# causalflow-ai/petit-kernel

Measured on AMD Instinct MI355X. Metric: bf16xnvfp4_gemm_achieved_hbm_bandwidth_m1_n8192_k8192, higher is better.
Workload: dtype bf16; 1 GPU; M=1 N=8192 K=8192 bf16 x nvfp4 (e4m3 scales, g=16), one mul_nvfp4_a16 call per step; weights_rotated_over_copies=37, parallelism=replicas x1 (no data-path collective), launch=hip graph replay (1 replays per region), statistic=one region, warmup_steps_run=4000

## Files before the change

### petit-kernel_amd/csrc/gemm_native32.hpp

```cpp
#pragma once

#include "gemm_native.hpp"
#include "gemm_wide.hpp"

#ifndef PETIT_ABLATE_N32
#define PETIT_ABLATE_N32 0
#endif

namespace petit_amd {

template <int ACT> __host__ __device__ inline size_t native32_ws_bytes(unsigned m, unsigned k) {
    return (size_t)m * (k / 8 * ACT) + (size_t)m * (k / 32);
}

struct QuantGather {
    const int *idx;
    unsigned a_rows, xb;
};
__device__ __forceinline__ unsigned q_row() { return blockIdx.y; }
__device__ __forceinline__ unsigned q_row(const QuantGather &g) { return blockIdx.x / g.xb; }
__device__ __forceinline__ unsigned q_bx() { return blockIdx.x; }
__device__ __forceinline__ unsigned q_bx(const QuantGather &g) { return blockIdx.x % g.xb; }
__device__ __forceinline__ unsigned q_src(unsigned row) { return row; }
__device__ __forceinline__ unsigned q_src(unsigned row, const QuantGather &g) { return g.idx ? (unsigned)g.idx[row] : row; }
// ... 295 lines not shown
    static constexpr int kSmemU4 = (kSmemU4a > kRedU4 ? kSmemU4a : kRedU4) + 16 * PW;
    static_assert(kSmemU4 * 16 <= 160 * 1024, "LDS budget");
    static constexpr int kMinWavesPerSimd = (kWantTwoPerSimd && (KG == 2 || kSmemU4 * 16 <= 80 * 1024)) ? 2 : 1;
};

constexpr int n32_stage_refills(bool last_span, int t_first, int kt, int d, int ks, int np, int wloads = 2) {
    if (t_first < 0)
        return wloads * np * kt;
    int n = 0;
    for (int t = t_first; t < t_first + kt; ++t)
        n += (!last_span || t + d < ks) ? wloads * np : 0;
    return n;
}

template <class Cfg, class... Moe>
__global__ __launch_bounds__(Cfg::kThreads, Cfg::kMinWavesPerSimd) void gemm_native32_kernel(const GemmArgs p, const unsigned char *ws,
                                                                                             const Moe... moe) {
    static_assert(sizeof...(Moe) <= 1, "at most one MoE locator");
    constexpr bool kIdx = sizeof...(Moe) == 1;
    using AT = typename Cfg::AT;
    constexpr int KS = Cfg::KS, MB = Cfg::MB, NP = Cfg::NP, WAVES = Cfg::WAVES, D = Cfg::D, ACT = Cfg::ACT;
    constexpr int KT = Cfg::KT, PF = Cfg::PF, NBUF = Cfg::NBUF, WM = Cfg::WM, kWaves = Cfg::kWaves;
    constexpr unsigned kRecBytes = ScaleRec<kFmtMx, KS>::kBytes;
    constexpr int kRecDw = ScaleRec<kFmtMx, KS>::kDwords;
    constexpr unsigned kOob = 0x80000000u;
    constexpr int kFragU4 = ACT == 4 ? 1 : 2;
    constexpr int kBlgp = ACT == 8 ? 0 : ACT == 6 ? 2 : 4;
    constexpr int WF = Cfg::WF, kWL = Cfg::kWLoads;
    constexpr int kCbsz = WF == 6 ? 2 : 4;

    __shared__ u32x4 smem[Cfg::kSmemU4];

    constexpr int KG = Cfg::KG;
    const unsigned tid = threadIdx.x;
    const unsigned lane = tid & 63u;
    const unsigned wave_all = __builtin_amdgcn_readfirstlane(tid >> 6);
    const unsigned kg = KG == 1 ? 0u : wave_all / kWaves;
    const unsigned wave = KG == 1 ? wave_all : wave_all % kWaves;
    const unsigned wn = WM == 1 ? wave : wave % WAVES, wm = WM == 1 ? 0u : wave / WAVES;
    const unsigned m_l = lane & 31u, h = lane >> 5;
    u32x4 *const smem_g = smem + kg * (NBUF * Cfg::kStageU4);

    const unsigned ktiles = p.k / kTileK;
    const unsigned nspans = ktiles / KS;
    const unsigned ntiles = p.n / kTileN;
    unsigned bn, bm, m0, m_lim = p.m;
    const void *w_e = p.w, *s_e = p.s, *bias_e = p.bias;
    const float *gs_e = p.gs;
    RowIndex ix{};
    if constexpr (kIdx) {
        if (!(moe.locate(p, bn, m0, m_lim, w_e, s_e, gs_e, bias_e, ix) && ...))
            return;
    } else {
        tile_of_block(p.flags, bn, bm);
    }
    const unsigned nt0 = (bn * WAVES + wn) * (2 * NP);
    if constexpr (!kIdx)
        m0 = bm * Cfg::BM;
    const unsigned part_begin = (blockIdx.z * KG + kg) * p.spans_per_wave;
    const bool empty_part = KG == 2 && part_begin >= nspans;
    const unsigned sp_begin = min(part_begin, nspans - 1);
    const unsigned sp_end = min(sp_begin + p.spans_per_wave, nspans);
    const unsigned kt_begin = sp_begin * KS;

    f32x16 acc[MB][NP];
#pragma unroll
    for (int mb = 0; mb < MB; ++mb)
#pragma unroll
        for (int np = 0; np < NP; ++np)
#pragma unroll
            for (int v = 0; v < 16; ++v)
                acc[mb][np][v] = 0.f;

    const unsigned valid_nt = (nt0 < ntiles && !empty_part) ? min((unsigned)(2 * NP), ntiles - nt0) : 0u;
    const unsigned w_row_bytes = ktiles * kTileBytes;
    const unsigned s_row_bytes = p.k / 2;
    const unsigned rows = min(m_lim - m0, (unsigned)Cfg::BM);
    const unsigned pt0 = valid_nt ? physical_tile(nt0, ntiles, p.act) : 0u;
    const unsigned span_tiles = !valid_nt ? 0u : p.act ? (valid_nt >> 1) + (ntiles >> 1) : valid_nt;
    const __amdgpu_buffer_rsrc_t w_rsrc = WF == 6 ? make_rsrc(w_e, (unsigned)nv6_elem_bytes(p.n, p.k))
                                                  : make_rsrc((const char *)w_e + (size_t)pt0 * w_row_bytes, span_tiles * w_row_bytes);
    const __amdgpu_buffer_rsrc_t s_rsrc = WF == 6 ? make_rsrc(s_e, (unsigned)nv6_scale_bytes(p.n, p.k))
                                                  : make_rsrc((const char *)s_e + (size_t)pt0 * s_row_bytes, span_tiles * s_row_bytes);
    unsigned w_voff[2 * NP], s_voff[2 * NP];
    if constexpr (WF == 6) {
#pragma unroll
        for (int np = 0; np < NP; ++np) {
            const unsigned nt = 2 * np + (m_l >> 4);
            const unsigned pt = physical_tile(nt0 + nt, ntiles, p.act);
            const unsigned lane_img = h * 32 + (pt & 1u) * 16 + (m_l & 15u);
            w_voff[np] = nt < valid_nt ? (pt >> 1) * (ktiles * kNv6TileBytes) + lane_img * 16 : kOob;
            s_voff[np] = nt < valid_nt ? (pt >> 1) * (ktiles * 128u) + lane_img * (2 * KS) : kOob;
        }
    } else {
#pragma unroll
        for (int nt = 0; nt < 2 * NP; ++nt) {
            const unsigned rel = physical_tile(nt0 + nt, ntiles, p.act) - pt0;
            w_voff[nt] = ((unsigned)nt < valid_nt) ? lane * 16 + rel * w_row_bytes : kOob;
            s_voff[nt] = ((unsigned)nt < valid_nt) ? lane * kRecBytes + rel * s_row_bytes : kOob;
        }
    }
    auto w_load = [&](int i, unsigned kt) -> u32x4 {
        if constexpr (WF == 6)
            return buf_load16(w_rsrc, w_voff[i / 3], kt * kNv6TileBytes + (i % 3) * 1024u, kAuxDefault);
        else
            return buf_load16(w_rsrc, w_voff[i], kt * kTileBytes, kAuxDefault);
    };
    constexpr unsigned kRowB = 16 * Cfg::kRowU4;
    const size_t qa_bytes = (size_t)p.m * (p.k / 8 * ACT), qs_bytes = (size_t)p.m * (p.k / 32);
    const size_t lo_bytes = (size_t)p.m * (p.k / 8 * Cfg::kRowU4);
    const __amdgpu_buffer_rsrc_t qa_rsrc = make_rsrc(ws + (size_t)m0 * kRowB, (unsigned)(lo_bytes - (size_t)m0 * kRowB));
    const __amdgpu_buffer_rsrc_t qh_rsrc = make_rsrc(ws + lo_bytes + (size_t)m0 * 32, ACT == 6 ? (unsigned)(qa_bytes - lo_bytes - (size_t)m0 * 32) : 0u);
    const __amdgpu_buffer_rsrc_t qs_rsrc = make_rsrc(ws + qa_bytes + (size_t)m0 * 4, (unsigned)(qs_bytes - (size_t)m0 * 4));
    const unsigned qa_tile = p.m * kRowB, qs_tile = p.m * 4;

    constexpr unsigned U = Cfg::kRowU4, RPL = Cfg::kRowsPerLoad;
    constexpr int kDmaWaves = Cfg::kDmaWaves;
    const bool dma_wave = kDmaWaves == kWaves || wave < (unsigned)kDmaWaves;
    const unsigned dma_row0 = wave * RPL + lane / U;
    auto swz = [](unsigned row) -> unsigned { return ACT == 8 ? (row >> 1) & 7u : (row >> 2) & 3u; };
    const unsigned hi_row0 = wave * 32 + (lane >> 1);
    const unsigned hi_voff = (ACT == 6 && dma_wave) ? hi_row0 * 32 + (((lane & 1u) ^ ((hi_row0 >> 3) & 1u)) * 16) : kOob;
    const unsigned dma_voff = dma_wave ? dma_row0 * kRowB + (((lane % U) ^ swz(dma_row0)) * 16) : kOob;
    const unsigned qs_voff = (wave * 64 < (unsigned)Cfg::BM) ? (wave * 64 + lane) * 4 : kOob;
    auto dma_stage = [&](unsigned kt, unsigned buf) {
#if defined(__HIP_DEVICE_COMPILE__) && !(PETIT_ABLATE_N32 & 1)
#pragma unroll
        for (int t = 0; t < KT; ++t) {
            u32x4 *const data = smem_g + buf * Cfg::kStageU4 + t * Cfg::kDataU4;
            u32x4 *const dump = smem_g + buf * Cfg::kStageU4 + KT * (Cfg::kDataU4 + Cfg::kScaleU4);
#pragma unroll
            for (int i = 0; i < Cfg::kDataLoads; ++i)
                __builtin_amdgcn_raw_ptr_buffer_load_lds(qa_rsrc, (__attribute__((address_space(3))) void *)(dma_wave ? data + (i * kDmaWaves + wave) * 64 : dump), 16,
                                                         dma_voff, i * (RPL * kDmaWaves) * kRowB + (kt + t) * qa_tile, 0, 0);
            if constexpr (ACT == 6) {
#pragma unroll
                for (int i = 0; i < Cfg::kHiLoads; ++i)
                    __builtin_amdgcn_raw_ptr_buffer_load_lds(qh_rsrc, (__attribute__((address_space(3))) void *)(dma_wave ? data + Cfg::kLoU4 + (i * kDmaWaves + wave) * 64 : dump), 16,
                                                             hi_voff, i * (32 * kDmaWaves) * 32 + (kt + t) * (p.m * 32), 0, 0);
            }
            u32x4 *const sc = smem_g + buf * Cfg::kStageU4 + KT * Cfg::kDataU4 + t * Cfg::kScaleU4;
            __builtin_amdgcn_raw_ptr_buffer_load_lds(qs_rsrc, (__attribute__((address_space(3))) void *)(sc + wave * 16), 4, qs_voff, (kt + t) * qs_tile, 0, 0);
        }
#else
        (void)kt, (void)buf;
#endif
    };
    struct Frags {
        u32x4 d[MB][kFragU4];
        int s[MB];
    };
    struct Frag1 {
        u32x4 d[kFragU4];
        int s;
    };
    const unsigned my_swz = swz(m_l);
    const unsigned hi_swz = (m_l >> 3) & 1u;
    auto read_frag1 = [&](const u32x4 *a_cur, const unsigned char *sc_bytes, int q, int mb, Frag1 &f) {
        const unsigned row = (wm * MB + mb) * 32 + m_l;
        if constexpr (ACT == 6) {
            f.d[0] = a_cur[row * U + ((2 * q + h) ^ my_swz)];
            if (q == 0)
                f.d[1] = a_cur[Cfg::kLoU4 + row * 2 + (h ^ hi_swz)];
        } else {
#pragma unroll
            for (int e = 0; e < kFragU4; ++e) {
                const unsigned unit = ACT == 8 ? 4 * q + 2 * h + e : 2 * q + h;
                f.d[e] = a_cur[row * U + (unit ^ my_swz)];
            }
        }
        f.s = (int)sc_bytes[row * 4 + 2 * q + h];
    };
    auto read_frags = [&](const u32x4 *a_cur, const unsigned char *sc_bytes, int q, Frags &f) {
#pragma unroll
        for (int mb = 0; mb < MB; ++mb) {
            const unsigned row = (wm * MB + mb) * 32 + m_l;
            if constexpr (ACT == 6) {
                f.d[mb][0] = a_cur[row * U + ((2 * q + h) ^ my_swz)];
                if (q == 0)
                    f.d[mb][1] = a_cur[Cfg::kLoU4 + row * 2 + (h ^ hi_swz)];
            } else {
#pragma unroll
                for (int e = 0; e < kFragU4; ++e) {
                    const unsigned unit = ACT == 8 ? 4 * q + 2 * h + e : 2 * q + h;
                    f.d[mb][e] = a_cur[row * U + (unit ^ my_swz)];
                }
            }
            f.s[mb] = (int)sc_bytes[row * 4 + 2 * q + h];
        }
// ... 30 lines not shown
#pragma unroll
            for (int i = 0; i < PF; ++i)
                load_stage(kt_begin + i * KT, i);
            asm volatile("s_waitcnt vmcnt(0)" ::: "memory");
            __builtin_amdgcn_s_barrier();
            const unsigned nstages = (sp_end - sp_begin) * (KS / KT);
            unsigned buf = PF % NBUF;
            for (unsigned st = 0; st < nstages; ++st) {
                load_stage(kt_begin + (st + PF) * KT, buf);
                buf = buf == (unsigned)(NBUF - 1) ? 0u : buf + 1;
                if (st + 1 < nstages) {
                    asm volatile("s_waitcnt vmcnt(%0)" ::"n"((PF - 1) * kLdStage) : "memory");
                    __builtin_amdgcn_s_barrier();
                }
            }
            asm volatile("s_waitcnt vmcnt(0)" ::: "memory");
#endif
            return;
        }
        if constexpr (Cfg::PW) {
            if (wave_all == (unsigned)(kWaves * KG + 1)) {
#if defined(__HIP_DEVICE_COMPILE__)
                constexpr int kPwTiles = 2 * NP * WAVES, kPwLoads = (kPwTiles * 8 + 63) / 64, kAhead = PETIT_N32_PW;
                const unsigned nt0_wg = bn * WAVES * (2 * NP);
                const unsigned valid_wg = nt0_wg < ntiles ? min((unsigned)kPwTiles, ntiles - nt0_wg) : 0u;
                const unsigned pt0_wg = valid_wg ? physical_tile(nt0_wg, ntiles, p.act) : 0u;
                const unsigned span_wg = !valid_wg ? 0u : p.act ? (valid_wg >> 1) + (ntiles >> 1) : valid_wg;
                const __amdgpu_buffer_rsrc_t pw_rsrc = make_rsrc((const char *)w_e + (size_t)pt0_wg * w_row_bytes, span_wg * w_row_bytes);
                u32x4 *const pw_dump = smem + (Cfg::kSmemU4 - 16);
                unsigned pvoff[kPwLoads];
#pragma unroll
                for (int j = 0; j < kPwLoads; ++j) {
                    const unsigned idx = j * 64 + lane, t = idx / 8, line = idx % 8;
                    const bool mine = PETIT_N32_PWSHARE == 1 || (idx % PETIT_N32_PWSHARE) == ((m0 / Cfg::BM) % PETIT_N32_PWSHARE);
                    pvoff[j] = (t < valid_wg && mine) ? (physical_tile(nt0_wg + t, ntiles, p.act) - pt0_wg) * w_row_bytes + line * 128 : kOob;
                }
                auto prefetch = [&](unsigned kt) {
                    if (kt < kt_end) {
#pragma unroll
                        for (int j = 0; j < kPwLoads; ++j)
                            __builtin_amdgcn_raw_ptr_buffer_load_lds(pw_rsrc, (__attribute__((address_space(3))) void *)pw_dump, 4, pvoff[j], kt * kTileBytes, 0, 0);
                    }
                };
                for (unsigned kt = kt_begin + D; kt < kt_begin + kAhead; ++kt)
                    prefetch(kt);
                __builtin_amdgcn_s_barrier();
                const unsigned nstages = (sp_end - sp_begin) * (KS / KT);
                for (unsigned st = 0; st < nstages; ++st) {
#pragma unroll
                    for (int t = 0; t < KT; ++t)
                        prefetch(kt_begin + st * KT + t + kAhead);
                    if (st + 1 < nstages)
                        __builtin_amdgcn_s_barrier();
                }
                asm volatile("s_waitcnt vmcnt(0)" ::: "memory");
#endif
                return;
            }
        }
    } else {
        dma_stage(kt_begin, 0);
#pragma unroll
        for (int i = 1; i < PF; ++i)
            if (kt_begin + i * KT < kt_end)
                dma_stage(kt_begin + i * KT, i);
    }
    ScaleRec<kFmtMx, KS> rec[NP][2], rec_next[NP][2];
    auto load_recs = [&](ScaleRec<kFmtMx, KS> (*dst)[2], unsigned sp) {
        if constexpr (WF == 6) {
#pragma unroll
            for (int np = 0; np < NP; ++np) {
                const ScaleRec<kFmtNv, KS> x = load_scale_rec<kFmtNv, KS>(s_rsrc, s_voff[np], sp * 64 * (2 * KS));
                if constexpr (KS == 2) {
                    dst[np][0].d[0] = x.d[0] & 0xffffu, dst[np][1].d[0] = x.d[0] >> 16;
                } else {
#pragma unroll
                    for (int d = 0; d < kRecDw; ++d)
                        dst[np][0].d[d] = x.d[d], dst[np][1].d[d] = x.d[kRecDw + d];
                }
            }
            return;
        }
#pragma unroll
        for (int np = 0; np < NP; ++np) {
            const ScaleRec<kFmtMx, KS> x = load_scale_rec<kFmtMx, KS>(s_rsrc, s_voff[2 * np], sp * 64 * kRecBytes);
            const ScaleRec<kFmtMx, KS> y = load_scale_rec<kFmtMx, KS>(s_rsrc, s_voff[2 * np + 1], sp * 64 * kRecBytes);
#pragma unroll
            for (int d = 0; d < kRecDw; ++d)
                merge_tiles(x.d[d], y.d[d], dst[np][0].d[d], dst[np][1].d[d]);
        }
    };
    load_recs(rec, sp_begin);
    u32x4 wring[D][kWL * NP];
#pragma unroll
    for (int i = 0; i < D; ++i)
#pragma unroll
        for (int nt = 0; nt < kWL * NP; ++nt)
            wring[i][nt] = w_load(nt, kt_begin + i);
    __syncthreads();

    unsigned cur_buf = 0;
    auto span_body = [&](const unsigned sp, auto last_c) {
        constexpr bool kLast = decltype(last_c)::value;
        const unsigned kt0 = sp * KS;
        if constexpr (!kLast)
            load_recs(rec_next, sp + 1);
        static_for<0, KS / KT>([&](auto s_c) {
            constexpr int S = decltype(s_c)::value, T0 = S * KT;
            constexpr bool kNextStage = !kLast || (T0 + KT < KS);
            const unsigned kt = kt0 + T0;
            const u32x4 *const stage = smem_g + cur_buf * Cfg::kStageU4;
            const unsigned char *const stage_sc = reinterpret_cast<const unsigned char *>(stage + KT * Cfg::kDataU4);
            if constexpr (PF == 1) {
                if constexpr (kNextStage)
                    dma_stage(kt + KT, cur_buf ^ 1u);
            } else {
                if constexpr (!Cfg::LW)
                    dma_stage(kt + PF * KT, cur_buf == 0 ? (unsigned)(NBUF - 1) : cur_buf - 1);
            }
            Frags fr[Cfg::kLean ? 1 : 2];
            Frag1 f1[2];
            unsigned tail_keep[MB][2];
            if constexpr (Cfg::kLean)
                read_frag1(stage, stage_sc, 0, 0, f1[0]);
            else
                read_frags(stage, stage_sc, 0, fr[0]);
            __builtin_amdgcn_sched_barrier(0);
            int refills = 0;
            static_for<0, KT>([&](auto t_c) {
                constexpr int TI = decltype(t_c)::value, T = T0 + TI, SLOT = T % D;
                constexpr bool kRefill = !kLast || (T + D < KS);
                const u32x4 *const a_cur = stage + TI * Cfg::kDataU4;
                const unsigned char *const sc_cur = stage_sc + TI * Cfg::kScaleU4 * 16;
                i32x8 wop[NP][2];
#pragma unroll
                for (int np = 0; np < NP; ++np) {
                    if constexpr (WF == 6) {
                        const u32x4 l1 = wring[SLOT][3 * np], l2 = wring[SLOT][3 * np + 1], tl = wring[SLOT][3 * np + 2];
                        wop[np][0] = i32x8{(int)l1[0], (int)l1[1], (int)l1[2], (int)l1[3], (int)tl[0], (int)tl[1], 0, 0};
                        wop[np][1] = i32x8{(int)l2[0], (int)l2[1], (int)l2[2], (int)l2[3], (int)tl[2], (int)tl[3], 0, 0};
                    } else {
                        unsigned pw[2][4];
#pragma unroll
                        for (int j = 0; j < 4; ++j)
                            merge_tiles(wring[SLOT][2 * np][j], wring[SLOT][2 * np + 1][j], pw[0][j], pw[1][j]);
#pragma unroll
                        for (int q = 0; q < 2; ++q)
                            wop[np][q] = i32x8{(int)pw[q][0], (int)pw[q][1], (int)pw[q][2], (int)pw[q][3], 0, 0, 0, 0};
                    }
                }
                auto refill_slot = [&]() {
                    if constexpr (kRefill && !(PETIT_ABLATE_N32 & 2)) {
#pragma unroll
                        for (int nt = 0; nt < kWL * NP; ++nt)
                            wring[SLOT][nt] = w_load(nt, kt0 + T + D);
                    }
                };
                if constexpr (WF != 6)
                    refill_slot();
                static_for<0, 2>([&](auto q_c) {
                    constexpr int q = decltype(q_c)::value, gi = 2 * TI + q;
                    if constexpr (Cfg::kLean) {
                        static_for<0, MB>([&](auto mb_c) {
                            constexpr int mb = decltype(mb_c)::value, li = gi * MB + mb;
                            if constexpr (li + 1 < 2 * KT * MB) {
                                constexpr int ngi = (li + 1) / MB, nmb = (li + 1) % MB, nti = ngi / 2, nq = ngi % 2;
                                read_frag1(stage + nti * Cfg::kDataU4, stage_sc + nti * Cfg::kScaleU4 * 16, nq, nmb, f1[(li + 1) & 1]);
                            }
                            const u32x4 lo = f1[li & 1].d[0], hi = f1[li & 1].d[kFragU4 - 1];
                            i32x8 aop;
                            if constexpr (ACT == 6) {
                                if constexpr (q == 0) {
                                    tail_keep[mb][0] = hi[2], tail_keep[mb][1] = hi[3];
                                    aop = i32x8{(int)lo[0], (int)lo[1], (int)lo[2], (int)lo[3], (int)hi[0], (int)hi[1], 0, 0};
                                } else {
                                    aop = i32x8{(int)lo[0], (int)lo[1], (int)lo[2], (int)lo[3], (int)tail_keep[mb][0], (int)tail_keep[mb][1], 0, 0};
                                }
                            } else {
                                aop = i32x8{(int)lo[0], (int)lo[1], (int)lo[2], (int)lo[3], (int)hi[0], (int)hi[1], (int)hi[2], (int)hi[3]};
                            }
#pragma unroll
                            for (int np = 0; np < NP; ++np)
                                acc[mb][np] = __builtin_amdgcn_mfma_scale_f32_32x32x64_f8f6f4(wop[np][q], aop, acc[mb][np], kCbsz , kBlgp ,
                                                                                              T % 4, (int)rec[np][q].d[T / 4], 0, f1[li & 1].s);
                        });
                    }
                    if constexpr (!Cfg::kLean && gi + 1 < 2 * KT && !(PETIT_ABLATE_N32 & 4)) {
                        constexpr int nti = (gi + 1) / 2, nq = (gi + 1) % 2;
                        read_frags(stage + nti * Cfg::kDataU4, stage_sc + nti * Cfg::kScaleU4 * 16, nq, fr[(gi + 1) & 1]);
                        if constexpr (ACT == 6 && nq == 1) {
#pragma unroll
                            for (int mb = 0; mb < MB; ++mb)
                                fr[1].d[mb][1] = fr[0].d[mb][1];
                        }
                    }
#pragma unroll
                    for (int mb = 0; mb < (Cfg::kLean ? 0 : MB); ++mb) {
                        i32x8 aop;
                        constexpr int fi = (PETIT_ABLATE_N32 & 4) ? 0 : (Cfg::kLean ? 0 : (gi & 1));
                        if constexpr (ACT == 8) {
                            const u32x4 lo = fr[fi].d[mb][0], hi = fr[fi].d[mb][kFragU4 - 1];
                            aop = i32x8{(int)lo[0], (int)lo[1], (int)lo[2], (int)lo[3], (int)hi[0], (int)hi[1], (int)hi[2], (int)hi[3]};
                        } else if constexpr (ACT == 6) {
                            const u32x4 lo = fr[fi].d[mb][0], tail = fr[fi].d[mb][1];
                            aop = i32x8{(int)lo[0], (int)lo[1], (int)lo[2], (int)lo[3], (int)tail[2 * q], (int)tail[2 * q + 1], 0, 0};
                        } else {
                            const u32x4 lo = fr[fi].d[mb][0];
                            aop = i32x8{(int)lo[0], (int)lo[1], (int)lo[2], (int)lo[3], 0, 0, 0, 0};
                        }
#pragma unroll
                        for (int np = 0; np < NP; ++np) {
                            if constexpr (PETIT_ABLATE_N32 & 8) {
#if defined(__HIP_DEVICE_COMPILE__)
                                asm volatile("" ::"v"(wop[np][q]), "v"(aop), "v"(fr[fi].s[mb]), "v"(rec[np][q].d[T / 4]));
#endif
                            } else {
                                acc[mb][np] = __builtin_amdgcn_mfma_scale_f32_32x32x64_f8f6f4(
                                    wop[np][q], aop, acc[mb][np], kCbsz , kBlgp , T % 4,
                                    (int)rec[np][q].d[T / 4], 0, fr[fi].s[mb]);
                            }
                        }
                    }
                    __builtin_amdgcn_sched_barrier(0);
                });
                if constexpr (WF == 6) {
                    refill_slot();
                    __builtin_amdgcn_sched_barrier(0);
                }
                (void)a_cur, (void)sc_cur, (void)refills;
            });
            if constexpr (PF == 1) {
                if constexpr (kNextStage)
                    __syncthreads();
                cur_buf ^= 1u;
            } else {
                if constexpr (kNextStage) {
                    constexpr int kPrevRefills = [] {
                        int n = 0;
                        for (int j = 1; j < PF; ++j)
                            n += n32_stage_refills(kLast, T0 - j * KT, KT, D, KS, NP, Cfg::kWLoads);
                        n += n32_stage_refills(kLast, T0, KT, D, KS, NP, Cfg::kWLoads);
                        return (PETIT_ABLATE_N32 & 2) ? 0 : n;
                    }();
#if defined(__HIP_DEVICE_COMPILE__)
                    if constexpr (!Cfg::LW)
                        asm volatile("s_waitcnt vmcnt(%0)" ::"n"((PF - 1) * Cfg::kStageLoads + kPrevRefills) : "memory");
                    __builtin_amdgcn_s_barrier();
#endif
                }
                __builtin_amdgcn_sched_barrier(0);
                cur_buf = cur_buf == (unsigned)(NBUF - 1) ? 0u : cur_buf + 1;
            }
            __builtin_amdgcn_sched_barrier(0);
        });
        if constexpr (!kLast) {
#pragma unroll
            for (int np = 0; np < NP; ++np)
                rec[np][0] = rec_next[np][0], rec[np][1] = rec_next[np][1];
        }
    };
    for (unsigned sp = sp_begin; sp + 1 < sp_end; ++sp)
        span_body(sp, std::false_type{});
    span_body(sp_end - 1, std::true_type{});

#pragma unroll
    for (int mb = 0; mb < MB; ++mb)
#pragma unroll
        for (int np = 0; np < NP; ++np) {
#if defined(__HIP_DEVICE_COMPILE__)
            asm volatile("" : "+v"(acc[mb][np]));
#endif
        }

    if constexpr (KG == 2) {
        for (unsigned i = sp_end - sp_begin; i < p.spans_per_wave; ++i)
            for (int b = 0; b < KS / KT; ++b)
                __builtin_amdgcn_s_barrier();
        __syncthreads();
        float *const red = reinterpret_cast<float *>(smem);
        if (kg == 1) {
#pragma unroll
            for (int mb = 0; mb < MB; ++mb)
#pragma unroll
                for (int np = 0; np < NP; ++np)
#pragma unroll
                    for (int v = 0; v < 16; ++v)
                        red[(((wn * MB + mb) * NP + np) * 16 + v) * 64 + lane] = acc[mb][np][v];
        }
        __syncthreads();
        if (kg == 0) {
#pragma unroll
            for (int mb = 0; mb < MB; ++mb)
#pragma unroll
                for (int np = 0; np < NP; ++np)
#pragma unroll
                    for (int v = 0; v < 16; ++v)
                        acc[mb][np][v] += red[(((wn * MB + mb) * NP + np) * 16 + v) * 64 + lane];
        }
    }

    if constexpr (PETIT_ABLATE_N32 & 16)
        return;
    const unsigned m_base = m0 + wm * (32 * MB) + m_l;
    if (gridDim.z > 1) {
        if (KG == 2 && kg != 0)
            return;
#pragma unroll
        for (int mb = 0; mb < MB; ++mb)
#pragma unroll
            for (int np = 0; np < NP; ++np)
#pragma unroll
// ... 73 lines not shown
```

### petit-kernel_amd/csrc/gemm_wide.hpp

```cpp
#pragma once

#include "gemm_tiled.hpp"

namespace petit_amd {

typedef __attribute__((ext_vector_type(16))) float f32x16;

#ifndef PETIT_ABLATE
#define PETIT_ABLATE 0
#endif

__device__ __forceinline__ f32x16 mfma32(bf16x8 a, bf16x8 b, f32x16 c) {
    return __builtin_amdgcn_mfma_f32_32x32x16_bf16(a, b, c, 0, 0, 0);
}
__device__ __forceinline__ f32x16 mfma32(f16x8 a, f16x8 b, f32x16 c) {
    return __builtin_amdgcn_mfma_f32_32x32x16_f16(a, b, c, 0, 0, 0);
}

__device__ __forceinline__ void pin_here(unsigned &x) {
#if defined(__HIP_DEVICE_COMPILE__)
    asm volatile("" : "+v"(x));
#endif
}
__device__ __forceinline__ void pin_here(u32x4 &x) {
// ... 4 lines not shown

__device__ __forceinline__ void merge_tiles(unsigned x, unsigned y, unsigned &p1, unsigned &p2) {
    const auto a = __builtin_amdgcn_permlane16_swap(x, y, false, false);
    const unsigned a0 = a[0], a1 = a[1];
    const auto b = __builtin_amdgcn_permlane32_swap(a0, a1, false, false);
    p1 = b[0], p2 = b[1];
}

template <class AT_, int FMT_, int KS_, int MB_, int NP_, int WAVES_, int D_, int PF_ = 1, int KG_ = 1, int GA_ = 0> struct WideCfg {
    using AT = AT_;
    static constexpr int GA = GA_;
    static_assert(GA_ == 0 || (KG_ == 1 && PF_ == 1 && !AT_::kAdaptive), "group-ahead form: one K group, double-buffered A tile, plain 16-bit activations");
    static constexpr int FMT = FMT_, KS = KS_, MB = MB_, NP = NP_, WAVES = WAVES_, D = D_, PF = PF_, NBUF = PF_ + 1, KG = KG_;
    static constexpr int kThreads = 64 * WAVES * KG;
    static constexpr int BM = 32 * MB, BN = 32 * NP * WAVES;
    static constexpr int kBufU4 = BM * 16;
    static constexpr int kDmaLoads = BM * 16 / 64 / WAVES;
    static constexpr int kMinWavesPerSimd = (KG == 2 || (NP == 1 && MB <= 4 && PF == 1)) ? 2 : 1;
    static constexpr int kRedU4 = KG == 2 ? BM * BN / 4 : 0;
    static constexpr int kSmemU4 = KG * NBUF * kBufU4 > kRedU4 ? KG * NBUF * kBufU4 : kRedU4;
    static_assert(KG == 1 || KG == 2, "one or two K groups");
    static_assert(PF == 1 || PF == 2, "prefetch distance 1 or 2");
    static_assert(!AT::kBfp, "plain bf16 / fp16 activations (or Fp16Mx: fast body + exact fallback, device_common.hpp)");
    static_assert(!AT::kAdaptive || FMT == kFmtMx, "Fp16Mx: fp16 activations x MXFP4 weights");
    static_assert(KS % D == 0, "ring depth must divide the span");
    static_assert((BM * 16) % (64 * WAVES) == 0 && (4 * WAVES) % 16 == 0, "A tile must split into whole 16-row groups per wave-load");
    static_assert(kSmemU4 * 16 <= 160 * 1024, "LDS budget");
};

template <class Cfg>
__global__ __launch_bounds__(Cfg::kThreads, Cfg::kMinWavesPerSimd) void gemm_wide_kernel(const GemmArgs p) {
    using AT = typename Cfg::AT;
    using Frag = typename AT::frag;
    constexpr int FMT = Cfg::FMT, KS = Cfg::KS, MB = Cfg::MB, NP = Cfg::NP, WAVES = Cfg::WAVES, D = Cfg::D;
    constexpr int PF = Cfg::PF, NBUF = Cfg::NBUF;
    constexpr unsigned kRecBytes = ScaleRec<FMT, KS>::kBytes;
    constexpr int kRecDw = ScaleRec<FMT, KS>::kDwords;
    constexpr unsigned kOob = 0x80000000u;

    constexpr int KG = Cfg::KG;
    __shared__ u32x4 smem_all[Cfg::kSmemU4];

    const unsigned tid = threadIdx.x;
    const unsigned lane = tid & 63u;
    const unsigned wave_all = __builtin_amdgcn_readfirstlane(tid >> 6);
    const unsigned kg = KG == 1 ? 0u : wave_all / WAVES;
    const unsigned wave = KG == 1 ? wave_all : wave_all % WAVES;
    u32x4 *const smem = smem_all + kg * (NBUF * Cfg::kBufU4);
    const unsigned m_l = lane & 31u, h = lane >> 5;

    const unsigned ktiles = p.k / kTileK;
    const unsigned nspans = ktiles / KS;
    const unsigned ntiles = p.n / kTileN;
    unsigned bn, bm;
    tile_of_block(p.flags, bn, bm);
    stagger_priority(p.flags);
    const unsigned nt0 = (bn * WAVES + wave) * (2 * NP);
    const unsigned m0 = bm * Cfg::BM;
    const unsigned part_begin = (blockIdx.z * KG + kg) * p.spans_per_wave;
    const bool empty_part = KG == 2 && part_begin >= nspans;
    const unsigned sp_begin = min(part_begin, nspans - 1);
    const unsigned sp_end = min(sp_begin + p.spans_per_wave, nspans);
    const unsigned kt_begin = sp_begin * KS;

    f32x16 acc[MB][NP];
#pragma unroll
    for (int mb = 0; mb < MB; ++mb)
#pragma unroll
        for (int np = 0; np < NP; ++np)
#pragma unroll
            for (int v = 0; v < 16; ++v)
                acc[mb][np][v] = 0.f;

    const unsigned valid_nt = (nt0 < ntiles && !empty_part) ? min((unsigned)(2 * NP), ntiles - nt0) : 0u;
    const unsigned w_row_bytes = ktiles * kTileBytes;
    const unsigned s_row_bytes = (FMT == kFmtNv) ? p.k : p.k / 2;
    const unsigned rows = min(p.m - m0, (unsigned)Cfg::BM);
    const unsigned pt0 = valid_nt ? physical_tile(nt0, ntiles, p.act) : 0u;
    const unsigned span_tiles = !valid_nt ? 0u : p.act ? (valid_nt >> 1) + (ntiles >> 1) : valid_nt;
    const __amdgpu_buffer_rsrc_t w_rsrc = make_rsrc((const char *)p.w + (size_t)pt0 * w_row_bytes, span_tiles * w_row_bytes);
    const __amdgpu_buffer_rsrc_t s_rsrc = make_rsrc((const char *)p.s + (size_t)pt0 * s_row_bytes, span_tiles * s_row_bytes);
    const __amdgpu_buffer_rsrc_t a_rsrc = make_rsrc((const char *)p.a + (size_t)m0 * p.k * 2, rows * p.k * 2);

    unsigned w_voff[2 * NP], s_voff[2 * NP];
#pragma unroll
    for (int nt = 0; nt < 2 * NP; ++nt) {
        const unsigned rel = physical_tile(nt0 + nt, ntiles, p.act) - pt0;
        w_voff[nt] = ((unsigned)nt < valid_nt) ? lane * 16 + rel * w_row_bytes : kOob;
        s_voff[nt] = ((unsigned)nt < valid_nt) ? lane * kRecBytes + rel * s_row_bytes : kOob;
    }
    const unsigned dma_row0 = wave * 4 + (lane >> 4);
    const unsigned dma_voff = dma_row0 * p.k * 2 + (((lane & 15u) ^ (dma_row0 & 15u)) * 16);
    auto dma_a_tile = [&](u32x4 *dst, unsigned kt) {
#pragma unroll
        for (int i = 0; i < Cfg::kDmaLoads; ++i) {
#if defined(__HIP_DEVICE_COMPILE__)
            __builtin_amdgcn_raw_ptr_buffer_load_lds(a_rsrc, (__attribute__((address_space(3))) void *)(dst + (i * WAVES + wave) * 64),
                                                     16, dma_voff, i * (4 * WAVES) * p.k * 2 + kt * 256, 0, 0);
#else
            (void)dst, (void)kt;
#endif
        }
    };
    const unsigned frag_row = m_l * 16, frag_swz = m_l & 15u;
    auto read_frags = [&](const u32x4 *a_cur, int g, u32x4 *dst) {
        const int q = g >> 2, j = g & 3;
#pragma unroll
        for (int mb = 0; mb < MB; ++mb)
            dst[mb] = a_cur[mb * 32 * 16 + frag_row + ((unsigned)(8 * q + 4 * h + j) ^ frag_swz)];
    };

    bool mx_fb = false;
    if constexpr (AT::kAdaptive) {
        const unsigned range = (sp_end - sp_begin) * 64u * kRecBytes;
        unsigned bad = 0;
#pragma unroll
        for (int nt = 0; nt < 2 * NP; ++nt) {
            if ((unsigned)nt >= valid_nt)
                continue;
            const unsigned row0 = s_voff[nt] - lane * kRecBytes + sp_begin * 64u * kRecBytes;
#pragma unroll 4
            for (unsigned base = 0; base < range; base += 1024u) {
                const unsigned off = base + lane * 16u;
                const u32x4 v = __builtin_bit_cast(u32x4, __builtin_amdgcn_raw_buffer_load_b128(s_rsrc, off < range ? row0 + off : kOob, 0, kAuxDefault));
                unsigned t = 0;
#pragma unroll
                for (int d = 0; d < 4; ++d) {
                    const unsigned x = v[d];
                    t |= (0x8C8C8C8Cu - x) | (x - 0x72727272u);
                }
                bad |= off < range ? t : 0u;
            }
        }
        mx_fb = __builtin_amdgcn_ballot_w64((bad & 0xE0E0E0E0u) != 0) != 0;
    }

    const unsigned kt_end = sp_end * KS;
    dma_a_tile(smem, kt_begin);
    if constexpr (PF == 2) {
        if (kt_begin + 1 < kt_end)
            dma_a_tile(smem + Cfg::kBufU4, kt_begin + 1);
    }
    if (AT::kAdaptive && mx_fb) {
        if constexpr (AT::kAdaptive) {
            __syncthreads();
            unsigned rel = 0;
#pragma unroll 1
            for (unsigned kt = kt_begin; kt < kt_end; ++kt) {
                const u32x4 *const a_cur = smem + rel * Cfg::kBufU4;
                if constexpr (PF == 1) {
                    if (kt + 1 < kt_end)
                        dma_a_tile(smem + (rel ^ 1u) * Cfg::kBufU4, kt + 1);
                } else {
                    dma_a_tile(smem + (rel == 0 ? 2u : rel - 1) * Cfg::kBufU4, kt + 2);
                }
#pragma unroll
                for (int np = 0; np < NP; ++np) {
                    const u32x4 x = buf_load16(w_rsrc, w_voff[2 * np], kt * kTileBytes, kAuxDefault);
                    const u32x4 y = buf_load16(w_rsrc, w_voff[2 * np + 1], kt * kTileBytes, kAuxDefault);
                    float sc[2];
#pragma unroll
                    for (int q = 0; q < 2; ++q) {
                        const unsigned tile = (lane >> 4) & 1u, src_lane = 16u * (2u * q + (lane >> 5)) + (lane & 15u);
                        const unsigned voff = s_voff[2 * np] == kOob ? kOob : s_voff[2 * np] - lane * kRecBytes + src_lane * kRecBytes + kt % KS;
                        const unsigned voff_y = s_voff[2 * np + 1] == kOob ? kOob : s_voff[2 * np + 1] - lane * kRecBytes + src_lane * kRecBytes + kt % KS;
                        const unsigned sb = __builtin_amdgcn_raw_buffer_load_b8(s_rsrc, tile ? voff_y : voff, (kt / KS) * 64 * kRecBytes, kAuxDefault);
                        sc[q] = __builtin_bit_cast(float, (sb & 0xffu) << 23);
                    }
#pragma unroll
                    for (int j = 0; j < 4; ++j) {
                        unsigned p[2];
                        merge_tiles(x[j], y[j], p[0], p[1]);
#pragma unroll
                        for (int q = 0; q < 2; ++q) {
                            const bf16x8 wb = unpack_mx(Bf16{}, p[q], sc[q]);
#pragma unroll
                            for (int mb = 0; mb < MB; ++mb) {
                                u32x4 hi, lo;
                                split_f16(a_cur[mb * 32 * 16 + frag_row + ((unsigned)(8 * q + 4 * h + j) ^ frag_swz)], hi, lo);
                                acc[mb][np] = mfma32(wb, __builtin_bit_cast(bf16x8, hi), acc[mb][np]);
                                acc[mb][np] = mfma32(wb, __builtin_bit_cast(bf16x8, lo), acc[mb][np]);
                            }
                        }
                    }
                }
                if (kt + 1 < kt_end)
                    __syncthreads();
                rel = rel + 1 == (unsigned)NBUF ? 0u : rel + 1;
            }
        }
    } else {
    ScaleRec<FMT, KS> rec[NP][2], rec_next[NP][2];
    auto load_recs = [&](ScaleRec<FMT, KS> (*dst)[2], unsigned sp) {
#pragma unroll
        for (int np = 0; np < NP; ++np) {
            const ScaleRec<FMT, KS> x = load_scale_rec<FMT, KS>(s_rsrc, s_voff[2 * np], sp * 64 * kRecBytes);
            const ScaleRec<FMT, KS> y = load_scale_rec<FMT, KS>(s_rsrc, s_voff[2 * np + 1], sp * 64 * kRecBytes);
#pragma unroll
            for (int d = 0; d < kRecDw; ++d)
                merge_tiles(x.d[d], y.d[d], dst[np][0].d[d], dst[np][1].d[d]);
        }
    };
    load_recs(rec, sp_begin);
    u32x4 wring[D][2 * NP];
#pragma unroll
    for (int i = 0; i < D; ++i)
#pragma unroll
        for (int nt = 0; nt < 2 * NP; ++nt)
            wring[i][nt] = buf_load16(w_rsrc, w_voff[nt], (kt_begin + i) * kTileBytes, kAuxDefault);

    if constexpr (Cfg::GA) {
    Frag wfg[2][NP];
    unsigned pw2[NP][4];
    auto unpack_ga = [&](auto c_c, auto slot_c, auto t_c, const ScaleRec<FMT, KS> (*rc)[2]) {
        constexpr int C = decltype(c_c)::value, SLOT = decltype(slot_c)::value, TS = decltype(t_c)::value, j = C % 4, q = C / 4;
#pragma unroll
        for (int np = 0; np < NP; ++np) {
            unsigned w;
            if constexpr (q == 0) {
                unsigned x = wring[SLOT][2 * np][j], y = wring[SLOT][2 * np + 1][j];
                pin_here(x), pin_here(y);
                merge_tiles(x, y, w, pw2[np][j]);
            } else {
                w = pw2[np][j];
                pin_here(w);
            }
            float s_lo, s_hi;
            tile_scales<FMT, KS, TS>(rc[np][q], s_lo, s_hi);
            Frag f;
            if constexpr (PETIT_ABLATE & 4)
                f = __builtin_bit_cast(Frag, u32x4{w, w ^ __builtin_bit_cast(unsigned, s_lo), w, __builtin_bit_cast(unsigned, s_hi)});
            else if constexpr (FMT == kFmtNv)
                f = unpack_nv(AT{}, w, j < 2 ? s_lo : s_hi);
            else
                f = unpack_mx(AT{}, w, s_lo);
            u32x4 fb = __builtin_bit_cast(u32x4, f);
            pin_here(fb);
            wfg[C & 1][np] = __builtin_bit_cast(Frag, fb);
        }
    };
    unpack_ga(std::integral_constant<int, 0>{}, std::integral_constant<int, 0>{}, std::integral_constant<int, 0>{}, rec);
    __syncthreads();
    auto span_body = [&](const unsigned sp, auto last_c) {
        constexpr bool kLast = decltype(last_c)::value;
        const unsigned kt0 = sp * KS;
        if constexpr (!kLast)
            load_recs(rec_next, sp + 1);
        static_for<0, KS>([&](auto t_c) {
            constexpr int T = decltype(t_c)::value;
            constexpr int SLOT = T % D, NSLOT = (T + 1) % D;
            constexpr bool kNext = !kLast || (T + 1 < KS);
            constexpr bool kRefill = !kLast || (T + D < KS);
            constexpr int TN = (T + 1) % KS;
            const unsigned kt = kt0 + T;
            const u32x4 *const a_cur = smem + (T & 1) * Cfg::kBufU4;
            u32x4 *const a_pf = smem + ((T + 1) & 1) * Cfg::kBufU4;
            if constexpr (kNext && !(PETIT_ABLATE & 1))
                dma_a_tile(a_pf, kt + 1);
            u32x4 fr[2][MB];
            read_frags(a_cur, 0, fr[0]);
            if constexpr (PETIT_ABLATE & 8)
                read_frags(a_cur, 1, fr[1]);
            __builtin_amdgcn_sched_barrier(0);
            static_for<0, 8>([&](auto g_c) {
                constexpr int g = decltype(g_c)::value;
                if constexpr (g + 1 < 8 && !(PETIT_ABLATE & 8))
                    read_frags(a_cur, g + 1, fr[(g + 1) & 1]);
#pragma unroll
                for (int mb = 0; mb < MB; ++mb)
#pragma unroll
                    for (int np = 0; np < NP; ++np)
                        acc[mb][np] = mfma32(wfg[g & 1][np], __builtin_bit_cast(Frag, fr[g & 1][mb]), acc[mb][np]);
                if constexpr (g + 1 < 8) {
                    unpack_ga(std::integral_constant<int, g + 1>{}, std::integral_constant<int, SLOT>{}, t_c, rec);
                } else if constexpr (kNext) {
                    if constexpr (TN == 0)
                        unpack_ga(std::integral_constant<int, 0>{}, std::integral_constant<int, NSLOT>{}, std::integral_constant<int, 0>{}, rec_next);
                    else
                        unpack_ga(std::integral_constant<int, 0>{}, std::integral_constant<int, NSLOT>{}, std::integral_constant<int, TN>{}, rec);
                }
                if constexpr (g == 2 && kRefill && !(PETIT_ABLATE & 2)) {
#pragma unroll
                    for (int nt = 0; nt < 2 * NP; ++nt)
                        wring[SLOT][nt] = buf_load16(w_rsrc, w_voff[nt], (kt + D) * kTileBytes, kAuxDefault);
                }
                __builtin_amdgcn_sched_barrier(0);
            });
            if constexpr (kNext && !(PETIT_ABLATE & 32))
                __syncthreads();
        });
        if constexpr (!kLast) {
#pragma unroll
            for (int np = 0; np < NP; ++np)
                rec[np][0] = rec_next[np][0], rec[np][1] = rec_next[np][1];
        }
    };
    for (unsigned sp = sp_begin; sp + 1 < sp_end; ++sp)
        span_body(sp, std::false_type{});
    span_body(sp_end - 1, std::true_type{});
    } else {
    Frag wf[2][NP][2][4];
    unsigned pw2[NP][4];
    auto unpack_chunk = [&](auto c_c, auto slot_c, auto buf_c, auto t_c, const ScaleRec<FMT, KS> (*rc)[2]) {
        constexpr int C = decltype(c_c)::value, SLOT = decltype(slot_c)::value, BUF = decltype(buf_c)::value;
        constexpr int TS = decltype(t_c)::value, j = C % 4, q = C / 4;
#pragma unroll
        for (int np = 0; np < NP; ++np) {
            unsigned w;
            if constexpr (q == 0) {
                unsigned x = wring[SLOT][2 * np][j], y = wring[SLOT][2 * np + 1][j];
                pin_here(x), pin_here(y);
                merge_tiles(x, y, w, pw2[np][j]);
            } else {
                w = pw2[np][j];
                pin_here(w);
            }
            float s_lo, s_hi;
            tile_scales<FMT, KS, TS>(rc[np][q], s_lo, s_hi);
            Frag f;
            if constexpr (PETIT_ABLATE & 4)
                f = __builtin_bit_cast(Frag, u32x4{w, w ^ __builtin_bit_cast(unsigned, s_lo), w, __builtin_bit_cast(unsigned, s_hi)});
            else if constexpr (FMT == kFmtNv)
                f = unpack_nv(AT{}, w, j < 2 ? s_lo : s_hi);
            else
                f = unpack_mx(AT{}, w, s_lo);
            u32x4 fb = __builtin_bit_cast(u32x4, f);
            pin_here(fb);
            wf[BUF][np][q][j] = __builtin_bit_cast(Frag, fb);
        }
    };
    static_for<0, 8>([&](auto c_c) {
        unpack_chunk(c_c, std::integral_constant<int, 0>{}, std::integral_constant<int, 0>{}, std::integral_constant<int, 0>{}, rec);
    });
    if (kt_begin + D < kt_end) {
#pragma unroll
        for (int nt = 0; nt < 2 * NP; ++nt)
            wring[0][nt] = buf_load16(w_rsrc, w_voff[nt], (kt_begin + D) * kTileBytes, kAuxDefault);
    }
    __syncthreads();

    unsigned rel3 = 0;
    auto span_body = [&](const unsigned sp, auto last_c) {
        constexpr bool kLast = decltype(last_c)::value;
        const unsigned kt0 = sp * KS;
        if constexpr (!kLast)
            load_recs(rec_next, sp + 1);
        static_for<0, KS>([&](auto t_c) {
            constexpr int T = decltype(t_c)::value;
            constexpr int CUR = T % 2, NXT = (T + 1) % 2;
            constexpr int NSLOT = (T + 1) % D;
            constexpr bool kNext = !kLast || (T + 1 < KS);
            constexpr bool kRefill = !kLast || (T + 1 + D < KS);
            constexpr int TN = (T + 1) % KS;
            const unsigned kt = kt0 + T;
            unsigned cur_buf, pf_buf;
            if constexpr (NBUF == 2) {
                cur_buf = T & 1, pf_buf = (T + 1) & 1;
            } else {
                cur_buf = rel3, pf_buf = rel3 == 0 ? 2u : rel3 - 1;
            }
            const u32x4 *const a_cur = smem + cur_buf * Cfg::kBufU4;
            u32x4 *const a_pf = smem + pf_buf * Cfg::kBufU4;
            if constexpr (PETIT_ABLATE & 1) {
            } else if constexpr (PF == 1) {
                if constexpr (kNext)
                    dma_a_tile(a_pf, kt + 1);
            } else {
                dma_a_tile(a_pf, kt + 2);
            }
            u32x4 fr[2][MB];
            read_frags(a_cur, 0, fr[0]);
            __builtin_amdgcn_sched_barrier(0);
            static_for<0, 8>([&](auto g_c) {
                constexpr int g = decltype(g_c)::value;
                if constexpr (g + 1 < 8 && !(PETIT_ABLATE & 8))
                    read_frags(a_cur, g + 1, fr[(g + 1) & 1]);
                constexpr int q = g >> 2, j = g & 3;
#pragma unroll
                for (int mb = 0; mb < MB; ++mb)
#pragma unroll
                    for (int np = 0; np < NP; ++np)
                        if constexpr (PETIT_ABLATE & 16) {
                            const u32x4 wb = __builtin_bit_cast(u32x4, wf[CUR][np][q][j]), ab = fr[(PETIT_ABLATE & 8) ? 0 : (g & 1)][mb];
                            acc[mb][np][g] += __builtin_bit_cast(float, wb[0] ^ ab[1]);
                        } else {
                            acc[mb][np] = mfma32(wf[CUR][np][q][j], __builtin_bit_cast(Frag, fr[(PETIT_ABLATE & 8) ? 0 : (g & 1)][mb]), acc[mb][np]);
                        }
                if constexpr (kNext) {
                    if constexpr (TN == 0)
                        unpack_chunk(g_c, std::integral_constant<int, NSLOT>{}, std::integral_constant<int, NXT>{},
                                     std::integral_constant<int, 0>{}, rec_next);
                    else
                        unpack_chunk(g_c, std::integral_constant<int, NSLOT>{}, std::integral_constant<int, NXT>{},
                                     std::integral_constant<int, TN>{}, rec);
                }
                __builtin_amdgcn_sched_barrier(0);
            });
            if constexpr (PF == 1) {
                if constexpr (kRefill && !(PETIT_ABLATE & 2)) {
#pragma unroll
                    for (int nt = 0; nt < 2 * NP; ++nt)
                        wring[NSLOT][nt] = buf_load16(w_rsrc, w_voff[nt], (kt + 1 + D) * kTileBytes, kAuxDefault);
                }
                if constexpr (kNext && !(PETIT_ABLATE & 1))
                    __syncthreads();
            } else {
                if constexpr (kNext) {
#if defined(__HIP_DEVICE_COMPILE__)
                    asm volatile("s_waitcnt vmcnt(%0)" ::"n"(Cfg::kDmaLoads) : "memory");
                    __builtin_amdgcn_s_barrier();
#endif
                }
                __builtin_amdgcn_sched_barrier(0);
                if constexpr (kRefill) {
#pragma unroll
                    for (int nt = 0; nt < 2 * NP; ++nt)
                        wring[NSLOT][nt] = buf_load16(w_rsrc, w_voff[nt], (kt + 1 + D) * kTileBytes, kAuxDefault);
                }
                rel3 = rel3 == 2 ? 0u : rel3 + 1;
            }
        });
        if constexpr (!kLast) {
#pragma unroll
            for (int np = 0; np < NP; ++np)
                rec[np][0] = rec_next[np][0], rec[np][1] = rec_next[np][1];
        }
    };
    for (unsigned sp = sp_begin; sp + 1 < sp_end; ++sp)
        span_body(sp, std::false_type{});
    span_body(sp_end - 1, std::true_type{});
    }
    }
    if constexpr (AT::kAdaptive) {
        static_for<0, 2>([&](auto pass) {
#pragma unroll
            for (int mb = 0; mb < MB; ++mb)
#pragma unroll
                for (int np = 0; np < NP; ++np)
                    mfma_join_pin(acc[mb][np]);
            if constexpr (decltype(pass)::value == 0)
                mfma_join_settle();
        });
    }

    if constexpr (KG == 2) {
        for (unsigned i = sp_end - sp_begin; i < p.spans_per_wave; ++i)
            for (int b = 0; b < KS; ++b)
                __builtin_amdgcn_s_barrier();
        __syncthreads();
        float *const red = reinterpret_cast<float *>(smem_all);
        if (kg == 1) {
#pragma unroll
            for (int mb = 0; mb < MB; ++mb)
#pragma unroll
                for (int np = 0; np < NP; ++np)
#pragma unroll
                    for (int v = 0; v < 16; ++v)
                        red[(((wave * MB + mb) * NP + np) * 16 + v) * 64 + lane] = acc[mb][np][v];
        }
        __syncthreads();
        if (kg == 1)
            return;
#pragma unroll
        for (int mb = 0; mb < MB; ++mb)
#pragma unroll
            for (int np = 0; np < NP; ++np)
#pragma unroll
                for (int v = 0; v < 16; ++v)
                    acc[mb][np][v] += red[(((wave * MB + mb) * NP + np) * 16 + v) * 64 + lane];
    }

    const unsigned m_base = m0 + m_l;
    if (gridDim.z > 1) {
#pragma unroll
        for (int mb = 0; mb < MB; ++mb)
#pragma unroll
            for (int np = 0; np < NP; ++np)
#pragma unroll
                for (int u = 0; u < 4; ++u) {
                    const unsigned m = m_base + mb * 32;
                    const unsigned nt = 2 * np + (u >> 1);
                    const unsigned n = (nt0 + nt) * 16 + (u & 1) * 8 + 4 * h;
                    if (m < p.m && nt < valid_nt)
                        *reinterpret_cast<f32x4 *>(p.workspace + ((size_t)blockIdx.z * p.m + m) * p.n + n) =
                            f32x4{acc[mb][np][4 * u], acc[mb][np][4 * u + 1], acc[mb][np][4 * u + 2], acc[mb][np][4 * u + 3]};
                }
        return;
    }
    const float gs = *p.gs;
    if (p.act) {
        const unsigned n_half = p.n >> 1;
#pragma unroll
        for (int mb = 0; mb < MB; ++mb)
#pragma unroll
            for (int np = 0; np < NP; ++np)
#pragma unroll
                for (int u = 0; u < 2; ++u) {
                    const unsigned m = m_base + mb * 32;
                    const unsigned n = ((nt0 + 2 * np) >> 1) * 16 + u * 8 + 4 * h;
                    const f32x16 &a = acc[mb][np];
// ... 25 lines not shown
```

Before: 4964 GB/s.

## Load pre-paired weight and scale lanes directly instead of merging two tile loads

```diff
diff --git a/petit-kernel_amd/csrc/gemm_native32.hpp b/petit-kernel_amd/csrc/gemm_native32.hpp
--- a/petit-kernel_amd/csrc/gemm_native32.hpp
+++ b/petit-kernel_amd/csrc/gemm_native32.hpp
@@ -401,7 +401,7 @@
                                                   : make_rsrc((const char *)w_e + (size_t)pt0 * w_row_bytes, span_tiles * w_row_bytes);
     const __amdgpu_buffer_rsrc_t s_rsrc = WF == 6 ? make_rsrc(s_e, (unsigned)nv6_scale_bytes(p.n, p.k))
                                                   : make_rsrc((const char *)s_e + (size_t)pt0 * s_row_bytes, span_tiles * s_row_bytes);
-    unsigned w_voff[2 * NP], s_voff[2 * NP];
+    unsigned w_voff[NP], s_voff[NP];
     if constexpr (WF == 6) {
 #pragma unroll
         for (int np = 0; np < NP; ++np) {
@@ -413,17 +413,19 @@
         }
     } else {
 #pragma unroll
-        for (int nt = 0; nt < 2 * NP; ++nt) {
+        for (int np = 0; np < NP; ++np) {
+            const unsigned nt = 2 * np + ((lane >> 4) & 1u);
             const unsigned rel = physical_tile(nt0 + nt, ntiles, p.act) - pt0;
-            w_voff[nt] = ((unsigned)nt < valid_nt) ? lane * 16 + rel * w_row_bytes : kOob;
-            s_voff[nt] = ((unsigned)nt < valid_nt) ? lane * kRecBytes + rel * s_row_bytes : kOob;
+            const unsigned unit = 16 * h + (lane & 15u);
+            w_voff[np] = nt < valid_nt ? unit * 16 + rel * w_row_bytes : kOob;
+            s_voff[np] = nt < valid_nt ? unit * kRecBytes + rel * s_row_bytes : kOob;
         }
     }
     auto w_load = [&](int i, unsigned kt) -> u32x4 {
         if constexpr (WF == 6)
             return buf_load16(w_rsrc, w_voff[i / 3], kt * kNv6TileBytes + (i % 3) * 1024u, kAuxDefault);
         else
-            return buf_load16(w_rsrc, w_voff[i], kt * kTileBytes, kAuxDefault);
+            return buf_load16(w_rsrc, w_voff[i / 2], kt * kTileBytes + (i % 2) * 512u, kAuxDefault);
     };
     constexpr unsigned kRowB = 16 * Cfg::kRowU4;
     const size_t qa_bytes = (size_t)p.m * (p.k / 8 * ACT), qs_bytes = (size_t)p.m * (p.k / 32);
@@ -620,13 +622,10 @@
             return;
         }
 #pragma unroll
-        for (int np = 0; np < NP; ++np) {
-            const ScaleRec<kFmtMx, KS> x = load_scale_rec<kFmtMx, KS>(s_rsrc, s_voff[2 * np], sp * 64 * kRecBytes);
-            const ScaleRec<kFmtMx, KS> y = load_scale_rec<kFmtMx, KS>(s_rsrc, s_voff[2 * np + 1], sp * 64 * kRecBytes);
-#pragma unroll
-            for (int d = 0; d < kRecDw; ++d)
-                merge_tiles(x.d[d], y.d[d], dst[np][0].d[d], dst[np][1].d[d]);
-        }
+        for (int np = 0; np < NP; ++np)
+#pragma unroll
+            for (int q = 0; q < 2; ++q)
+                dst[np][q] = load_scale_rec<kFmtMx, KS>(s_rsrc, s_voff[np], sp * 64 * kRecBytes + q * 32 * kRecBytes);
     };
     load_recs(rec, sp_begin);
     u32x4 wring[D][kWL * NP];
@@ -678,13 +677,11 @@
                         wop[np][0] = i32x8{(int)l1[0], (int)l1[1], (int)l1[2], (int)l1[3], (int)tl[0], (int)tl[1], 0, 0};
                         wop[np][1] = i32x8{(int)l2[0], (int)l2[1], (int)l2[2], (int)l2[3], (int)tl[2], (int)tl[3], 0, 0};
                     } else {
-                        unsigned pw[2][4];
-#pragma unroll
-                        for (int j = 0; j < 4; ++j)
-                            merge_tiles(wring[SLOT][2 * np][j], wring[SLOT][2 * np + 1][j], pw[0][j], pw[1][j]);
-#pragma unroll
-                        for (int q = 0; q < 2; ++q)
-                            wop[np][q] = i32x8{(int)pw[q][0], (int)pw[q][1], (int)pw[q][2], (int)pw[q][3], 0, 0, 0, 0};
+#pragma unroll
+                        for (int q = 0; q < 2; ++q) {
+                            const u32x4 l = wring[SLOT][2 * np + q];
+                            wop[np][q] = i32x8{(int)l[0], (int)l[1], (int)l[2], (int)l[3], 0, 0, 0, 0};
+                        }
                     }
                 }
                 auto refill_slot = [&]() {
@@ -694,8 +691,6 @@
                             wring[SLOT][nt] = w_load(nt, kt0 + T + D);
                     }
                 };
-                if constexpr (WF != 6)
-                    refill_slot();
                 static_for<0, 2>([&](auto q_c) {
                     constexpr int q = decltype(q_c)::value, gi = 2 * TI + q;
                     if constexpr (Cfg::kLean) {
@@ -761,10 +756,8 @@
                     }
                     __builtin_amdgcn_sched_barrier(0);
                 });
-                if constexpr (WF == 6) {
-                    refill_slot();
-                    __builtin_amdgcn_sched_barrier(0);
-                }
+                refill_slot();
+                __builtin_amdgcn_sched_barrier(0);
                 (void)a_cur, (void)sc_cur, (void)refills;
             });
             if constexpr (PF == 1) {
diff --git a/petit-kernel_amd/csrc/gemm_wide.hpp b/petit-kernel_amd/csrc/gemm_wide.hpp
--- a/petit-kernel_amd/csrc/gemm_wide.hpp
+++ b/petit-kernel_amd/csrc/gemm_wide.hpp
@@ -110,13 +110,31 @@
     const __amdgpu_buffer_rsrc_t s_rsrc = make_rsrc((const char *)p.s + (size_t)pt0 * s_row_bytes, span_tiles * s_row_bytes);
     const __amdgpu_buffer_rsrc_t a_rsrc = make_rsrc((const char *)p.a + (size_t)m0 * p.k * 2, rows * p.k * 2);
 
-    unsigned w_voff[2 * NP], s_voff[2 * NP];
-#pragma unroll
-    for (int nt = 0; nt < 2 * NP; ++nt) {
-        const unsigned rel = physical_tile(nt0 + nt, ntiles, p.act) - pt0;
-        w_voff[nt] = ((unsigned)nt < valid_nt) ? lane * 16 + rel * w_row_bytes : kOob;
-        s_voff[nt] = ((unsigned)nt < valid_nt) ? lane * kRecBytes + rel * s_row_bytes : kOob;
-    }
+    constexpr int kVoffs = Cfg::GA ? 2 * NP : NP;
+    unsigned w_voff[kVoffs], s_voff[kVoffs];
+    if constexpr (Cfg::GA) {
+#pragma unroll
+        for (int nt = 0; nt < 2 * NP; ++nt) {
+            const unsigned rel = physical_tile(nt0 + nt, ntiles, p.act) - pt0;
+            w_voff[nt] = ((unsigned)nt < valid_nt) ? lane * 16 + rel * w_row_bytes : kOob;
+            s_voff[nt] = ((unsigned)nt < valid_nt) ? lane * kRecBytes + rel * s_row_bytes : kOob;
+        }
+    } else {
+#pragma unroll
+        for (int np = 0; np < NP; ++np) {
+            const unsigned nt = 2 * np + ((lane >> 4) & 1u);
+            const unsigned rel = physical_tile(nt0 + nt, ntiles, p.act) - pt0;
+            const unsigned unit = 16 * h + (lane & 15u);
+            w_voff[np] = nt < valid_nt ? unit * 16 + rel * w_row_bytes : kOob;
+            s_voff[np] = nt < valid_nt ? unit * kRecBytes + rel * s_row_bytes : kOob;
+        }
+    }
+    auto w_load = [&](int i, unsigned kt) -> u32x4 {
+        if constexpr (Cfg::GA)
+            return buf_load16(w_rsrc, w_voff[i], kt * kTileBytes, kAuxDefault);
+        else
+            return buf_load16(w_rsrc, w_voff[i / 2], kt * kTileBytes + (i % 2) * 512u, kAuxDefault);
+    };
     const unsigned dma_row0 = wave * 4 + (lane >> 4);
     const unsigned dma_voff = dma_row0 * p.k * 2 + (((lane & 15u) ^ (dma_row0 & 15u)) * 16);
     auto dma_a_tile = [&](u32x4 *dst, unsigned kt) {
@@ -146,7 +164,7 @@
         for (int nt = 0; nt < 2 * NP; ++nt) {
             if ((unsigned)nt >= valid_nt)
                 continue;
-            const unsigned row0 = s_voff[nt] - lane * kRecBytes + sp_begin * 64u * kRecBytes;
+            const unsigned row0 = (physical_tile(nt0 + nt, ntiles, p.act) - pt0) * s_row_bytes + sp_begin * 64u * kRecBytes;
 #pragma unroll 4
             for (unsigned base = 0; base < range; base += 1024u) {
                 const unsigned off = base + lane * 16u;
@@ -184,24 +202,18 @@
                 }
 #pragma unroll
                 for (int np = 0; np < NP; ++np) {
-                    const u32x4 x = buf_load16(w_rsrc, w_voff[2 * np], kt * kTileBytes, kAuxDefault);
-                    const u32x4 y = buf_load16(w_rsrc, w_voff[2 * np + 1], kt * kTileBytes, kAuxDefault);
+                    const u32x4 pw[2] = {w_load(2 * np, kt), w_load(2 * np + 1, kt)};
                     float sc[2];
 #pragma unroll
                     for (int q = 0; q < 2; ++q) {
-                        const unsigned tile = (lane >> 4) & 1u, src_lane = 16u * (2u * q + (lane >> 5)) + (lane & 15u);
-                        const unsigned voff = s_voff[2 * np] == kOob ? kOob : s_voff[2 * np] - lane * kRecBytes + src_lane * kRecBytes + kt % KS;
-                        const unsigned voff_y = s_voff[2 * np + 1] == kOob ? kOob : s_voff[2 * np + 1] - lane * kRecBytes + src_lane * kRecBytes + kt % KS;
-                        const unsigned sb = __builtin_amdgcn_raw_buffer_load_b8(s_rsrc, tile ? voff_y : voff, (kt / KS) * 64 * kRecBytes, kAuxDefault);
+                        const unsigned sb = __builtin_amdgcn_raw_buffer_load_b8(s_rsrc, s_voff[np], (kt / KS) * 64 * kRecBytes + q * 32 * kRecBytes + kt % KS, kAuxDefault);
                         sc[q] = __builtin_bit_cast(float, (sb & 0xffu) << 23);
                     }
 #pragma unroll
                     for (int j = 0; j < 4; ++j) {
-                        unsigned p[2];
-                        merge_tiles(x[j], y[j], p[0], p[1]);
 #pragma unroll
                         for (int q = 0; q < 2; ++q) {
-                            const bf16x8 wb = unpack_mx(Bf16{}, p[q], sc[q]);
+                            const bf16x8 wb = unpack_mx(Bf16{}, pw[q][j], sc[q]);
 #pragma unroll
                             for (int mb = 0; mb < MB; ++mb) {
                                 u32x4 hi, lo;
@@ -222,11 +234,17 @@
     auto load_recs = [&](ScaleRec<FMT, KS> (*dst)[2], unsigned sp) {
 #pragma unroll
         for (int np = 0; np < NP; ++np) {
-            const ScaleRec<FMT, KS> x = load_scale_rec<FMT, KS>(s_rsrc, s_voff[2 * np], sp * 64 * kRecBytes);
-            const ScaleRec<FMT, KS> y = load_scale_rec<FMT, KS>(s_rsrc, s_voff[2 * np + 1], sp * 64 * kRecBytes);
-#pragma unroll
-            for (int d = 0; d < kRecDw; ++d)
-                merge_tiles(x.d[d], y.d[d], dst[np][0].d[d], dst[np][1].d[d]);
+            if constexpr (Cfg::GA) {
+                const ScaleRec<FMT, KS> x = load_scale_rec<FMT, KS>(s_rsrc, s_voff[2 * np], sp * 64 * kRecBytes);
+                const ScaleRec<FMT, KS> y = load_scale_rec<FMT, KS>(s_rsrc, s_voff[2 * np + 1], sp * 64 * kRecBytes);
+#pragma unroll
+                for (int d = 0; d < kRecDw; ++d)
+                    merge_tiles(x.d[d], y.d[d], dst[np][0].d[d], dst[np][1].d[d]);
+            } else {
+#pragma unroll
+                for (int q = 0; q < 2; ++q)
+                    dst[np][q] = load_scale_rec<FMT, KS>(s_rsrc, s_voff[np], sp * 64 * kRecBytes + q * 32 * kRecBytes);
+            }
         }
     };
     load_recs(rec, sp_begin);
@@ -235,7 +253,7 @@
     for (int i = 0; i < D; ++i)
 #pragma unroll
         for (int nt = 0; nt < 2 * NP; ++nt)
-            wring[i][nt] = buf_load16(w_rsrc, w_voff[nt], (kt_begin + i) * kTileBytes, kAuxDefault);
+            wring[i][nt] = w_load(nt, kt_begin + i);
 
     if constexpr (Cfg::GA) {
     Frag wfg[2][NP];
@@ -328,21 +346,13 @@
     span_body(sp_end - 1, std::true_type{});
     } else {
     Frag wf[2][NP][2][4];
-    unsigned pw2[NP][4];
     auto unpack_chunk = [&](auto c_c, auto slot_c, auto buf_c, auto t_c, const ScaleRec<FMT, KS> (*rc)[2]) {
         constexpr int C = decltype(c_c)::value, SLOT = decltype(slot_c)::value, BUF = decltype(buf_c)::value;
         constexpr int TS = decltype(t_c)::value, j = C % 4, q = C / 4;
 #pragma unroll
         for (int np = 0; np < NP; ++np) {
-            unsigned w;
-            if constexpr (q == 0) {
-                unsigned x = wring[SLOT][2 * np][j], y = wring[SLOT][2 * np + 1][j];
-                pin_here(x), pin_here(y);
-                merge_tiles(x, y, w, pw2[np][j]);
-            } else {
-                w = pw2[np][j];
-                pin_here(w);
-            }
+            unsigned w = wring[SLOT][2 * np + q][j];
+            pin_here(w);
             float s_lo, s_hi;
             tile_scales<FMT, KS, TS>(rc[np][q], s_lo, s_hi);
             Frag f;
@@ -363,7 +373,7 @@
     if (kt_begin + D < kt_end) {
 #pragma unroll
         for (int nt = 0; nt < 2 * NP; ++nt)
-            wring[0][nt] = buf_load16(w_rsrc, w_voff[nt], (kt_begin + D) * kTileBytes, kAuxDefault);
+            wring[0][nt] = w_load(nt, kt_begin + D);
     }
     __syncthreads();
 
@@ -428,7 +438,7 @@
                 if constexpr (kRefill && !(PETIT_ABLATE & 2)) {
 #pragma unroll
                     for (int nt = 0; nt < 2 * NP; ++nt)
-                        wring[NSLOT][nt] = buf_load16(w_rsrc, w_voff[nt], (kt + 1 + D) * kTileBytes, kAuxDefault);
+                        wring[NSLOT][nt] = w_load(nt, kt + 1 + D);
                 }
                 if constexpr (kNext && !(PETIT_ABLATE & 1))
                     __syncthreads();
@@ -443,7 +453,7 @@
                 if constexpr (kRefill) {
 #pragma unroll
                     for (int nt = 0; nt < 2 * NP; ++nt)
-                        wring[NSLOT][nt] = buf_load16(w_rsrc, w_voff[nt], (kt + 1 + D) * kTileBytes, kAuxDefault);
+                        wring[NSLOT][nt] = w_load(nt, kt + 1 + D);
                 }
                 rel3 = rel3 == 2 ? 0u : rel3 + 1;
             }
```

Result: no change. 4952 GB/s (-0.2%).
